# td-kwj-zp2023/webgpu-msm-twisted-edwards

Hardware: AMD Instinct MI355X
Metric: MSMs/sec at n=2^20 Twisted-Edwards BLS12 (pipelined throughput = 1000/ms_per_step; single-MSM latency in latency_ms) (higher is better)
Workload: dtype u32

## Files before the change

webgpu-msm-twisted-edwards_amd/csrc/curve.hpp:

```cpp
#pragma once
#include "field.hpp"

namespace te {

template <int N> struct ete_t { fel<N> x, y, z, t; };
using ete = ete_t<9>;

template <int N> struct pnt_t;
template <> struct pnt_t<9> { fel<9> hm, hp, dt; };
template <> struct pnt_t<14> { fel<14> hm, hp, dt, z; };
using pnt = pnt_t<9>;
struct pnt_aff377 { fel<14> hm, hp, dt; };

template <int N> TE_HD ete_t<N> ete_identity_t() { ete_t<N> r; r.x = fe_zero<N>(); r.y = fe_one<N>(); r.z = fe_one<N>(); r.t = fe_zero<N>(); return r; }
TE_HD ete ete_identity() { return ete_identity_t<9>(); }

TE_HD uint32_t mask_select(uint32_t m, uint32_t b, uint32_t a) {
#if defined(__HIP_DEVICE_COMPILE__)
  return __builtin_amdgcn_bitop3_b32(m, b, a, 0xCA);
#else
  return (b & m) | (a & ~m);
#endif
}
template <int N> TE_HD pnt_t<N> pnt_cneg(const pnt_t<N>& a, bool neg) {
  pnt_t<N> r = a; const fel<N> ndt = fe_neg<4>(a.dt);
  const uint32_t m = neg ? 0xffffffffu : 0u;
#pragma unroll
  for (int i = 0; i < N; i++) {
    r.hm.v[i] = mask_select(m, a.hp.v[i], a.hm.v[i]);
    r.hp.v[i] = mask_select(m, a.hm.v[i], a.hp.v[i]);
    r.dt.v[i] = mask_select(m, ndt.v[i], a.dt.v[i]);
  }
  return r;
}

TE_HD pnt_aff377 pnt_cneg(const pnt_aff377& a, bool neg) {
  pnt_aff377 r = a; const fel<14> ndt = fe_neg<4>(a.dt);
  const uint32_t m = neg ? 0xffffffffu : 0u;
#pragma unroll
  for (int i = 0; i < 14; i++) {
    r.hm.v[i] = mask_select(m, a.hp.v[i], a.hm.v[i]);
    r.hp.v[i] = mask_select(m, a.hm.v[i], a.hp.v[i]);
    r.dt.v[i] = mask_select(m, ndt.v[i], a.dt.v[i]);
  }
  return r;
}

template <bool MONT = false> TE_HD pnt pnt_from_affine_raw(const fp& x, const fp& y) {
  const fp k = MONT ? fp_R2_HALF_A() : fp_R2_HALF();
  const fp a[2] = {fp_sub<16>(y, x), fp_add(y, x)}, b[2] = {k, k};
  fp o[2];
  mont_mul_x<2>(a, b, o);
  pnt r;
  r.hm = o[0]; r.hp = o[1];
  r.dt = fp_mul_d(mont_mul(fp_add(o[1], o[0]), fp_sub<2>(o[0], o[1])));
  return r;
}

template <bool MONT = false> TE_HD pnt_t<14> pnt_from_sw377(const fel<14>& x, const fel<14>& y) {
  using namespace te377;
  const fq a1[3] = {x, y, x}, b1[3] = {MONT ? fq_S_R2_A() : fq_S_R2(), MONT ? fq_R2_A() : fq_R2(), MONT ? fq_F_R2_A() : fq_F_R2()};
  fq o1[3];
  fe_mul_x<3>(a1, b1, o1);
  const fq w = fe_norm(fe_add(o1[0], fq_SP1_MONT())), bb = fe_add(o1[0], fq_SM1_MONT()), aa = fe_norm(fe_add(o1[2], fq_F_MONT()));
  const fq a2[4] = {w, o1[1], o1[1], aa}, b2[4] = {aa, bb, w, bb};
  fq o2[4];
  fe_mul_x<4>(a2, b2, o2);
  pnt_t<14> r;
  r.hm = fe_norm(fe_sub<2>(o2[1], o2[0]));
  r.hp = fe_norm(fe_add(o2[1], o2[0]));
  r.z = fe_norm(fe_add(o2[2], o2[2]));
  r.dt = fe_mul(o2[3], fq_NEG_2D_MONT());
  return r;
}

template <int N> TE_HD ete_t<N> ete_close(const fel<N>& E, const fel<N>& H, const fel<N>& F, const fel<N>& G) {
  const fel<N> En = fe_norm_if_needed(E), Gn = fe_norm_if_needed(G);
  const fel<N> l[4] = {En, H, En, Gn}, rr[4] = {F, Gn, H, F};
  fel<N> o[4];
  fe_mul_x<4>(l, rr, o);
  ete_t<N> r;
  r.x = o[0]; r.y = o[1]; r.t = o[2]; r.z = o[3];
  return r;
}

TE_HD ete ete_madd(const ete& a, const pnt& b) {
  const fp in1[3] = {fp_sub<2>(a.y, a.x), fp_add(a.y, a.x), a.t}, in2[3] = {b.hm, b.hp, b.dt};
  fp abc[3];
  mont_mul_x<3>(in1, in2, abc);
  const fp &A = abc[0], &B = abc[1], &Cn = abc[2];
  return ete_close<9>(fp_sub<2>(B, A), fp_add(B, A), fp_add(a.z, Cn), fp_sub<2>(a.z, Cn));
}
TE_HD ete_t<14> ete_madd(const ete_t<14>& a, const pnt_t<14>& b) {
  const fel<14> in1[4] = {fe_sub<2>(a.y, a.x), fe_add(a.y, a.x), a.t, a.z}, in2[4] = {b.hm, b.hp, b.dt, b.z};
  fel<14> p[4];
  fe_mul_x<4>(in1, in2, p);
  const fel<14> &A = p[0], &B = p[1], &Cn = p[2], &D = p[3];
  return ete_close<14>(fe_sub<2>(B, A), fe_add(B, A), fe_add(D, Cn), fe_sub<2>(D, Cn));
}

TE_HD ete_t<14> ete_madd(const ete_t<14>& a, const pnt_aff377& b) {
  const fel<14> in1[3] = {fe_sub<2>(a.y, a.x), fe_add(a.y, a.x), a.t}, in2[3] = {b.hm, b.hp, b.dt};
  fel<14> p[3];
  fe_mul_x<3>(in1, in2, p);
  const fel<14> &A = p[0], &B = p[1], &Cn = p[2];
  return ete_close<14>(fe_sub<2>(B, A), fe_add(B, A), fe_add(a.z, Cn), fe_sub<2>(a.z, Cn));
}

TE_HD ete ete_from_pnt(const pnt& b) {
  const fp one = fp_R1();
  const fp E = fp_sub<2>(b.hp, b.hm), H = fp_add(b.hp, b.hm);
  const fp l[3] = {E, H, E}, rr[3] = {one, one, H};
  fp o[3];
  mont_mul_x<3>(l, rr, o);
  ete r;
  r.x = o[0]; r.y = o[1]; r.t = o[2]; r.z = one;
  return r;
}
TE_HD ete_t<14> ete_from_pnt(const pnt_t<14>& b) {
  const fel<14> En = fe_norm(fe_sub<2>(b.hp, b.hm)), H = fe_add(b.hp, b.hm);
  const fel<14> l[4] = {En, H, En, b.z}, rr[4] = {b.z, b.z, H, b.z};
  fel<14> o[4];
  fe_mul_x<4>(l, rr, o);
  ete_t<14> r;
  r.x = o[0]; r.y = o[1]; r.t = o[2]; r.z = o[3];
  return r;
}

TE_HD ete_t<14> ete_from_pnt(const pnt_aff377& b) {
  const fel<14> one = fe_one<14>();
  const fel<14> En = fe_norm(fe_sub<2>(b.hp, b.hm)), H = fe_add(b.hp, b.hm);
  const fel<14> l[3] = {En, H, En}, rr[3] = {one, one, H};
  fel<14> o[3];
  fe_mul_x<3>(l, rr, o);
  ete_t<14> r;
  r.x = o[0]; r.y = o[1]; r.t = o[2]; r.z = one;
  return r;
}

TE_HD ete ete_from_pair(const pnt& a, const pnt& b) {
  const fp one = fp_R1();
  const fp T1 = mont_mul(fp_add(a.hp, a.hm), fp_sub<2>(a.hp, a.hm));
  const fp in1[3] = {fp_add(a.hm, a.hm), fp_add(a.hp, a.hp), T1}, in2[3] = {b.hm, b.hp, b.dt};
  fp abc[3];
  mont_mul_x<3>(in1, in2, abc);
  const fp &A = abc[0], &B = abc[1], &Cn = abc[2];
  return ete_close<9>(fp_sub<2>(B, A), fp_add(B, A), fp_add(one, Cn), fp_sub<2>(one, Cn));
}
TE_HD ete_t<14> ete_from_pair(const pnt_aff377& a, const pnt_aff377& b) {
  const fel<14> one = fe_one<14>();
  const fel<14> T1 = fe_mul(fe_add(a.hp, a.hm), fe_norm(fe_sub<2>(a.hp, a.hm)));
  const fel<14> in1[3] = {fe_add(a.hm, a.hm), fe_add(a.hp, a.hp), T1}, in2[3] = {b.hm, b.hp, b.dt};
  fel<14> p[3];
  fe_mul_x<3>(in1, in2, p);
  const fel<14> &A = p[0], &B = p[1], &Cn = p[2];
  return ete_close<14>(fe_sub<2>(B, A), fe_add(B, A), fe_add(one, Cn), fe_sub<2>(one, Cn));
}
TE_HD ete_t<14> ete_from_pair(const pnt_t<14>& a, const pnt_t<14>& b) { return ete_madd(ete_from_pnt(a), b); }

template <int N> TE_HD ete_t<N> ete_add(const ete_t<N>& a, const ete_t<N>& b) {
  const fel<N> in1[4] = {fe_norm(fe_sub<2>(a.y, a.x)), fe_norm_if_needed(fe_add(a.y, a.x)), a.t, a.z};
  const fel<N> in2[4] = {fe_sub<2>(b.y, b.x), fe_add(b.y, b.x), b.t, b.z};
  fel<N> p1[4];
  fe_mul_x<4>(in1, in2, p1);
  const fel<N> &A = p1[0], &B = p1[1];
  const fel<N> C = fe_mul_k2d(p1[2]);
  const fel<N> D = fe_add(p1[3], p1[3]);
  const fel<N> E = fe_norm_if_needed(fe_sub<2>(B, A));
  const fel<N> H = fe_add(B, A);
  const fel<N> F = fe_norm(fe_sub<2>(D, C));
  const fel<N> G = fe_norm_if_needed(fe_add(D, C));
  const fel<N> l[4] = {E, H, E, F}, rr[4] = {F, G, H, G};
  fel<N> o[4];
  fe_mul_x<4>(l, rr, o);
  ete_t<N> r;
  r.x = o[0]; r.y = o[1]; r.t = o[2]; r.z = o[3];
  return r;
}

}
```

webgpu-msm-twisted-edwards_amd/csrc/kernels.hip.hpp:

```cpp
#pragma once
#include <hip/hip_runtime.h>
#include "curve.hpp"
#include "scalar_form.hpp"

namespace te {

#define TE_BATCH_MAX 8
struct batch_ptrs { const uint4* p[TE_BATCH_MAX]; };
struct batch_slabs { uint32_t s[TE_BATCH_MAX]; };

struct digits_params {
  uint32_t half[10];
  uint32_t zero_digit;
  uint32_t sc_stride;
  uint32_t n, nst;
  int num_windows;
  int w_first, w_step, nw_local;
  uint32_t half_code, logS, P, CH, chunk_len;
};

struct pnt_slot { uint4 q[8]; };
template <bool MONT = false>
__device__ __forceinline__ void prep_points_block(uint32_t blk, uint4* __restrict__ lds, const uint4* __restrict__ pts, pnt_slot* __restrict__ recs, uint32_t n) {
  const uint32_t t = threadIdx.x, base = blk * 256u;
// ... 363 lines not shown
      }
    }
    __syncthreads();
    for (uint32_t p = t; p < g.P; p += 512u) { run_base[p] += tile_cnt[p]; tile_cnt[p] = 0u; }
    __syncthreads();
  }
}

__global__ void __launch_bounds__(512) k_part_scatter(scatter_args a) {
  __shared__ uint32_t lds[TE_SCATTER_LDS_WORDS];
  part_scatter_block<false>(blockIdx.x, blockIdx.y, lds, a, index_args{});
}
__global__ void __launch_bounds__(512) k_part_scatter_indexed(scatter_args a, index_args x) {
  __shared__ uint32_t lds[TE_SCATTER_LDS_WORDS];
  part_scatter_block<true>(blockIdx.x, blockIdx.y, lds, a, x);
}

#ifndef TE_SCATTER_PREP_WAVES
#define TE_SCATTER_PREP_WAVES 8
#endif
__global__ void __launch_bounds__(512, TE_SCATTER_PREP_WAVES) k_part_scatter_prep(scatter_args a, uint32_t scatter_blocks, batch_ptrs in, batch_slabs row_slab,
                                                           pnt_slot* __restrict__ recs, uint32_t n, uint32_t prep_blocks_per_row, uint32_t prep_blocks) {
  __shared__ uint4 lds4[(TE_SCATTER_LDS_WORDS + 3u) / 4u > 256u * 8u ? (TE_SCATTER_LDS_WORDS + 3u) / 4u : 256u * 8u];
  const uint64_t tot = (uint64_t)scatter_blocks + prep_blocks, b = blockIdx.x;
  const uint32_t s_before = (uint32_t)(b * scatter_blocks / tot), s_after = (uint32_t)((b + 1u) * scatter_blocks / tot);
  if (s_after > s_before) {
    part_scatter_block<false>(s_before % a.g.CH, s_before / a.g.CH, reinterpret_cast<uint32_t*>(lds4), a, index_args{});
  } else {
    const uint32_t pb = (uint32_t)b - s_before, row = pb / prep_blocks_per_row, blk = pb - row * prep_blocks_per_row;
    prep_points_block(blk, lds4, in.p[row], recs + (size_t)row_slab.s[row] * n, n);
  }
}


struct piece_regs { uint4 k[5], ia[5], ib[5]; };
template <bool PK>
__device__ __forceinline__ void load_piece(const uint16_t* __restrict__ keys_row, const uint32_t* __restrict__ idx_row, uint32_t a, uint32_t b,
                                           uint32_t t, bool with_idx, piece_regs& r, uint32_t& head, uint32_t& total) {
  const uint32_t a_al = a & ~7u;
  head = a - a_al; total = head + (b - a);
  const uint32_t groups = (total + 7u) >> 3;
  const uint4* k4 = reinterpret_cast<const uint4*>(keys_row + a_al);
  const uint4* i4 = reinterpret_cast<const uint4*>(idx_row + a_al);
#pragma unroll
  for (int c = 0; c < 5; c++) {
    const uint32_t gi = min((uint32_t)c * 256u + t, groups - 1u);
    if (!PK) r.k[c] = k4[gi];
    if (PK || with_idx) { r.ia[c] = i4[2 * gi]; r.ib[c] = i4[2 * gi + 1]; }
  }
}
template <bool PK> __device__ __forceinline__ void piece_group(const piece_regs& r, int c, uint32_t (&kv)[8], uint32_t (&iv)[8]) {
  const uint32_t w[8] = {r.ia[c].x, r.ia[c].y, r.ia[c].z, r.ia[c].w, r.ib[c].x, r.ib[c].y, r.ib[c].z, r.ib[c].w};
  if (PK) {
#pragma unroll
    for (int e = 0; e < 8; e++) { kv[e] = ((w[e] >> 23) & 0xffu) | ((w[e] >> 31) << 15); iv[e] = w[e] & 0x7fffffu; }
  } else {
    unpack8(r.k[c], kv);
#pragma unroll
    for (int e = 0; e < 8; e++) iv[e] = w[e];
  }
}
static_assert(5u * 256u * 8u >= TE_L2_CAP + 8u, "five groups per thread hold a piece");

__device__ __forceinline__ bool l2_piece_of_block(uint32_t bx, const uint32_t* __restrict__ pc, uint32_t P, uint32_t overflow_pieces, uint32_t* sm, uint32_t* pj, uint32_t& p, uint32_t& j) {
  if (bx < P) { p = bx; j = 0u; return true; }
  const uint32_t t = threadIdx.x, x = bx - P;
  if (x >= overflow_pieces) return false;
  const uint32_t c = t < P ? pc[t] : 0u;
  const uint32_t ov = c ? (c + TE_L2_CAP - 1u) / TE_L2_CAP - 1u : 0u;
  uint32_t tot;
  const uint32_t ex = block_excl_scan(ov, sm, tot);
  if (x >= tot) return false;
  if (x >= ex && x < ex + ov) { pj[0] = t; pj[1] = x - ex + 1u; }
  __syncthreads();
  p = pj[0]; j = pj[1];
  __syncthreads();
  return true;
}

#define TE_COMBINE_SMALL 16u
#define TE_GIANT_RUN 256u
#define TE_SEG_INVALID 0xffffffffu
#define TE_HIST_COPIES 32u
struct plan_args {
  const uint32_t* part_start; const uint32_t* part_count; const uint32_t* seg_part_base;
  uint32_t *bucket_start, *bucket_cursor, *seg_base, *seg_bucket, *seg_lenv, *size_hist, *split_list;
  uint32_t* split_count;
  uint32_t* chunk_list;
  uint32_t seg_len, cap_w, chunk_cap;
};
struct plan_lds { uint32_t h[1024]; uint32_t sm[17]; uint32_t giant[256 * 3]; uint32_t n_giant; };
__device__ __forceinline__ uint32_t seg_plan_block(uint32_t p, uint32_t k, uint32_t cnt_in, const sort_geom& sg, const plan_args& a, plan_lds& L,
                                                   uint32_t pstart, uint32_t pcount, uint32_t sbase) {
  const uint32_t t = threadIdx.x, P = sg.P, S = sg.S, B = sg.B, seg_len = a.seg_len;
  uint32_t* const h = L.h; uint32_t* const sm = L.sm; uint32_t* const giant = L.giant;
  __syncthreads();
  for (uint32_t j = t; j < 1024u; j += 256u) h[j] = 0u;
  if (t == 0) L.n_giant = 0u;
  const bool mine = t < S;
  const uint32_t g = k * B + p * S + (mine ? t : 0u);
  const uint32_t cnt = mine ? cnt_in : 0u;
  const uint32_t nparts = mine ? max(1u, (cnt + seg_len - 1u) / seg_len) : 0u;
  uint32_t bt, bt2;
  const uint32_t ex = block_excl_scan(cnt, sm, bt);
  const uint32_t ex2 = block_excl_scan(nparts, sm, bt2);
  const uint32_t bs = pstart + ex, sb = sbase + ex2;
  if (mine) {
    a.bucket_start[g] = bs; a.bucket_cursor[g] = bs; a.seg_base[g] = sb;
    if (nparts <= TE_COMBINE_SMALL) {
      for (uint32_t part = 0; part < nparts; part++) {
        const uint32_t len = cnt > part * seg_len ? min(seg_len, cnt - part * seg_len) : 0u;
        a.seg_bucket[sb + part] = g; a.seg_lenv[sb + part] = len;
        atomicAdd(&h[min(len, 1023u)], 1u);
      }
      if (nparts > 1u) a.split_list[atomicAdd(&a.split_count[0], 1u)] = g;
    } else {
      const uint32_t j = atomicAdd(&L.n_giant, 1u);
      giant[3 * j] = g; giant[3 * j + 1] = sb; giant[3 * j + 2] = cnt;
      atomicAdd(&a.split_count[1], 1u);
    }
  }
  {
    const uint32_t first = sbase, used = bt2;
    const uint32_t cap = p + 1u == P ? (k + 1u) * a.cap_w - first : S + pcount / seg_len;
    for (uint32_t j = used + t; j < cap; j += 256u) { a.seg_bucket[first + j] = TE_SEG_INVALID; a.seg_lenv[first + j] = TE_SEG_INVALID; }
  }
  __syncthreads();
  const uint32_t ng = L.n_giant;
  for (uint32_t j = 0; j < ng; j++) {
    const uint32_t gg = giant[3 * j], sb0 = giant[3 * j + 1], c0 = giant[3 * j + 2];
    const uint32_t np = (c0 + seg_len - 1u) / seg_len;
    for (uint32_t part = t; part < np; part += 256u) {
      const uint32_t len = min(seg_len, c0 - part * seg_len);
      a.seg_bucket[sb0 + part] = gg; a.seg_lenv[sb0 + part] = len;
      atomicAdd(&h[min(len, 1023u)], 1u);
      if ((part & (TE_GIANT_RUN - 1u)) == 0) { const uint32_t ci = atomicAdd(&a.split_count[2], 1u); if (ci < a.chunk_cap) { a.chunk_list[2 * ci] = gg; a.chunk_list[2 * ci + 1] = part; } }
    }
  }
  __syncthreads();
  uint32_t* my_hist = a.size_hist + ((k * P + p) % TE_HIST_COPIES) * 1024u;
  for (uint32_t j = t; j < 1024u; j += 256u) if (h[j]) atomicAdd(&my_hist[j], h[j]);
  __syncthreads();
  return ex;
}

struct l2_args {
  const uint16_t* part_keys; const uint32_t* part_idx; const uint32_t* part_start; const uint32_t* part_count;
  uint32_t* bucket_count; uint32_t* sorted;
  uint32_t* part_ticket;
  sort_geom g; plan_args pa;
};
#define TE_L2A_LDS_WORDS (3u * 256u + 32u + TE_L2_LIST)
static_assert(sizeof(plan_lds) <= TE_L2_LIST * 4u, "the plan's LDS fits into the list area");
template <bool PK>
__global__ void __launch_bounds__(256, TE_L2_WAVES) k_l2_local(l2_args a) {
  __shared__ uint32_t lds[TE_L2A_LDS_WORDS];
  uint32_t* const cnt_s = lds; uint32_t* const off_s = lds + 256; uint32_t* const sm = lds + 768; uint32_t* const pj = lds + 768 + 17;
  uint32_t* const list = lds + 768 + 32;
  plan_lds& PL = *reinterpret_cast<plan_lds*>(list);
  const sort_geom& g = a.g;
  const uint32_t k = gridDim.y - 1u - blockIdx.y, t = threadIdx.x;
  const uint32_t extra = gridDim.x - g.P, bx = blockIdx.x < extra ? g.P + blockIdx.x : blockIdx.x - extra;
  const uint32_t* ps = a.part_start + k * g.P; const uint32_t* pc = a.part_count + k * g.P;
  uint32_t p, j;
  if (!l2_piece_of_block(bx, pc, g.P, bx < g.P ? 0u : a.part_count[gridDim.y * g.P + k], sm, pj, p, j)) return;
  const uint32_t cntp = pc[p], pb = ps[p], sbp = a.pa.seg_part_base[k * g.P + p];
  if (cntp == 0u) { (void)seg_plan_block(p, k, 0u, g, a.pa, PL, pb, cntp, sbp); return; }
  const bool single = cntp <= TE_L2_CAP;
  const uint32_t a0 = pb + j * TE_L2_CAP, b0 = min(pb + cntp, a0 + TE_L2_CAP);
  const uint16_t* keys_row = a.part_keys + (size_t)k * g.nst; const uint32_t* idx_row = a.part_idx + (size_t)k * g.nst;
  piece_regs r; uint32_t head, total;
  load_piece<PK>(keys_row, idx_row, a0, b0, t, single, r, head, total);
  cnt_s[t] = 0u;
  __syncthreads();
#pragma unroll
  for (int c = 0; c < 5; c++) {
    uint32_t kv[8], iv[8]; piece_group<PK>(r, c, kv, iv);
    const uint32_t e0 = ((uint32_t)c * 256u + t) * 8u;
#pragma unroll
    for (int e = 0; e < 8; e++) { const uint32_t pos = e0 + (uint32_t)e; if (pos >= head && pos < total) atomicAdd(&cnt_s[kv[e] & 0x7fffu], 1u); }
  }
  __syncthreads();
  const uint32_t c0 = cnt_s[t];
  const size_t gb = (size_t)k * g.B + (size_t)p * g.S + t;
  if (!single) {
    if (c0) atomicAdd(&a.bucket_count[gb], c0);
    wait_own_accesses();
    __syncthreads();
    if (t == 0) pj[2] = (handoff_arrive(&a.part_ticket[k * g.P + p]) + 1u == (cntp + TE_L2_CAP - 1u) / TE_L2_CAP) ? 1u : 0u;
    __syncthreads();
    if (pj[2]) (void)seg_plan_block(p, k, t < g.S ? ld_agent(a.bucket_count + gb) : 0u, g, a.pa, PL, pb, cntp, sbp);
    return;
  }
  if (t < g.S) a.bucket_count[gb] = c0;
  const uint32_t ex = seg_plan_block(p, k, c0, g, a.pa, PL, pb, cntp, sbp);
  if (t < g.S) a.pa.bucket_cursor[gb] = pb + ex + c0;
  off_s[t] = ex;
  __syncthreads();
#pragma unroll
  for (int c = 0; c < 5; c++) {
    uint32_t kv[8], iv[8]; piece_group<PK>(r, c, kv, iv);
    const uint32_t e0 = ((uint32_t)c * 256u + t) * 8u;
#pragma unroll
    for (int e = 0; e < 8; e++) {
      const uint32_t pos = e0 + (uint32_t)e;
      if (pos >= head && pos < total) list[atomicAdd(&off_s[kv[e] & 0x7fffu], 1u)] = iv[e] | ((kv[e] >> 15) << 31);
    }
  }
  __syncthreads();
  uint32_t* out = a.sorted + (size_t)k * g.n + pb;
  for (uint32_t s = t; s < cntp; s += 256u) out[s] = list[s];
}

#define TE_ORDER_REGS 32u
__device__ __forceinline__ void order_scatter_block(uint32_t ob, uint32_t nob, uint32_t* __restrict__ lds, const uint32_t* __restrict__ lenv, uint32_t ids,
                                                    const uint32_t* __restrict__ size_hist, uint32_t* __restrict__ rel_cursor,
                                                    uint32_t* __restrict__ order, uint32_t* __restrict__ num_segments, uint32_t max_len) {
  uint32_t* const h = lds; uint32_t* const base = lds + 1024; uint32_t* const sm = lds + 2048;
  const uint32_t per = (ids + nob - 1) / nob;
  const uint32_t lo = min(ids, ob * per), hi = min(ids, lo + per);
  const bool in_regs = per <= TE_ORDER_REGS * 256u;
  uint32_t lv[TE_ORDER_REGS];
  if (in_regs) {
#pragma unroll
    for (uint32_t j = 0; j < TE_ORDER_REGS; j++) { const uint32_t g = lo + j * 256u + threadIdx.x; lv[j] = g < hi ? lenv[g] : TE_SEG_INVALID; }
  }
  for (uint32_t j = threadIdx.x; j < 1024u; j += 256u) h[j] = 0;
  {
    uint32_t run = 0;
    for (uint32_t c = (1023u - min(max_len, 1023u)) >> 8; c < 4u; c++) {
      const uint32_t s = 1023u - (c * 256u + threadIdx.x);
      uint32_t part[TE_HIST_COPIES];
#pragma unroll
      for (uint32_t r = 0; r < TE_HIST_COPIES; r++) part[r] = size_hist[r * 1024u + s];
      uint32_t cnt_s = 0;
#pragma unroll
      for (uint32_t r = 0; r < TE_HIST_COPIES; r++) cnt_s += part[r];
      uint32_t bt;
      const uint32_t ex = block_excl_scan(cnt_s, sm, bt);
      base[s] = run + ex;
      run += bt;
    }
    if (ob == 0 && threadIdx.x == 0) *num_segments = run;
  }
  __syncthreads();
  if (in_regs) {
#pragma unroll
    for (uint32_t j = 0; j < TE_ORDER_REGS; j++) if (lv[j] != TE_SEG_INVALID) atomicAdd(&h[min(lv[j], 1023u)], 1u);
  } else {
    for (uint32_t g = lo + threadIdx.x; g < hi; g += 256u) { const uint32_t l = lenv[g]; if (l != TE_SEG_INVALID) atomicAdd(&h[min(l, 1023u)], 1u); }
  }
  __syncthreads();
  for (uint32_t j = threadIdx.x; j < 1024u; j += 256u) { base[j] += h[j] ? atomicAdd(&rel_cursor[j], h[j]) : 0u; h[j] = 0; }
  __syncthreads();
  if (in_regs) {
#pragma unroll
    for (uint32_t j = 0; j < TE_ORDER_REGS; j++) {
      if (lv[j] == TE_SEG_INVALID) continue;
      const uint32_t sz = min(lv[j], 1023u);
      order[base[sz] + atomicAdd(&h[sz], 1u)] = lo + j * 256u + threadIdx.x;
    }
  } else {
    for (uint32_t g = lo + threadIdx.x; g < hi; g += 256u) {
      const uint32_t l = lenv[g];
      if (l == TE_SEG_INVALID) continue;
      const uint32_t sz = min(l, 1023u);
      order[base[sz] + atomicAdd(&h[sz], 1u)] = g;
    }
  }
}

#define TE_PLACE_LDS_WORDS (4u * 256u + TE_L2_LIST + TE_L2_LIST / 4u + 2u + 17u)
template <bool PK>
__device__ __forceinline__ void l2_place_piece(uint32_t p, uint32_t k, uint32_t a0, uint32_t b0, uint32_t* __restrict__ lds,
                                               const uint16_t* __restrict__ part_keys, const uint32_t* __restrict__ part_idx,
                                               uint32_t* __restrict__ bucket_cursor, uint32_t* __restrict__ sorted, const sort_geom& g) {
  uint32_t* const cnt_s = lds; uint32_t* const lex_s = lds + 256; uint32_t* const off_s = lds + 512; uint32_t* const gbase_s = lds + 768;
  uint32_t* const list = lds + 1024;
  uint8_t* const list_b = reinterpret_cast<uint8_t*>(list + TE_L2_LIST);
  uint32_t* const sm = list + TE_L2_LIST + TE_L2_LIST / 4u + 2u;
  const uint32_t t = threadIdx.x, len = b0 - a0;
  const uint16_t* keys_row = part_keys + (size_t)k * g.nst; const uint32_t* idx_row = part_idx + (size_t)k * g.nst;
  uint32_t* out = sorted + (size_t)k * g.n;
  cnt_s[t] = 0u;
  __syncthreads();
  piece_regs r; uint32_t head, total;
  load_piece<PK>(keys_row, idx_row, a0, b0, t, true, r, head, total);
#pragma unroll
  for (int c = 0; c < 5; c++) {
    uint32_t kv[8], iv[8]; piece_group<PK>(r, c, kv, iv);
    const uint32_t e0 = ((uint32_t)c * 256u + t) * 8u;
#pragma unroll
    for (int e = 0; e < 8; e++) { const uint32_t pos = e0 + (uint32_t)e; if (pos >= head && pos < total) atomicAdd(&cnt_s[kv[e] & 0x7fffu], 1u); }
  }
  __syncthreads();
  wave0_excl_scan(cnt_s, lex_s, 256u, &sm[16]);
  {
    const uint32_t c0 = cnt_s[t];
    gbase_s[t] = c0 ? atomicAdd(&bucket_cursor[(size_t)k * g.B + (size_t)p * g.S + t], c0) : 0u;
  }
  __syncthreads();
  off_s[t] = lex_s[t];
  gbase_s[t] -= lex_s[t];
  __syncthreads();
#pragma unroll
  for (int c = 0; c < 5; c++) {
    uint32_t kv[8], iv[8]; piece_group<PK>(r, c, kv, iv);
    const uint32_t e0 = ((uint32_t)c * 256u + t) * 8u;
#pragma unroll
    for (int e = 0; e < 8; e++) {
      const uint32_t pos = e0 + (uint32_t)e;
      if (pos >= head && pos < total) {
        const uint32_t b = kv[e] & 0x7fffu;
        const uint32_t slot = atomicAdd(&off_s[b], 1u);
        list[slot] = iv[e] | ((kv[e] >> 15) << 31); list_b[slot] = (uint8_t)b;
      }
    }
  }
  __syncthreads();
  for (uint32_t s = t; s < len; s += 256u) out[gbase_s[list_b[s]] + s] = list[s];
}

struct order_args { const uint32_t* lenv; uint32_t ids; const uint32_t* size_hist; uint32_t* rel_cursor; uint32_t* order; uint32_t* num_segments; uint32_t order_cols, max_len; };
template <bool PK>
__global__ void __launch_bounds__(256, TE_L2_WAVES) k_l2_place_order(const uint16_t* __restrict__ part_keys, const uint32_t* __restrict__ part_idx,
                                                           const uint32_t* __restrict__ part_start, const uint32_t* __restrict__ part_count,
                                                           uint32_t* __restrict__ bucket_cursor, uint32_t* __restrict__ sorted, sort_geom g, order_args oa) {
  __shared__ uint32_t lds[TE_PLACE_LDS_WORDS];
  if (blockIdx.x < oa.order_cols) {
    order_scatter_block(blockIdx.y * oa.order_cols + blockIdx.x, gridDim.y * oa.order_cols, lds, oa.lenv, oa.ids, oa.size_hist, oa.rel_cursor, oa.order, oa.num_segments, oa.max_len);
    return;
  }
  const uint32_t k = gridDim.y - 1u - blockIdx.y;
  const uint32_t px = blockIdx.x - oa.order_cols, extra = gridDim.x - oa.order_cols - g.P, bx = px < extra ? g.P + px : px - extra;
  const uint32_t* pc = part_count + k * g.P;
  uint32_t p, j;
  if (!l2_piece_of_block(bx, pc, g.P, bx < g.P ? 0u : part_count[gridDim.y * g.P + k], lds, lds + 32, p, j)) return;
  const uint32_t cntp = pc[p], pb = part_start[k * g.P + p];
  if (cntp <= TE_L2_CAP) return;
  const uint32_t a0 = pb + j * TE_L2_CAP;
  l2_place_piece<PK>(p, k, a0, min(pb + cntp, a0 + TE_L2_CAP), lds, part_keys, part_idx, bucket_cursor, sorted, g);
}

template <int N> struct geo {
  static constexpr uint32_t PW = 4u * N;
  static constexpr uint32_t PQ = PW / 4u;
  static constexpr uint32_t RW = N == 9 ? 27u : 4u * N;
  static constexpr uint32_t SQ = N == 9 ? 8u : N;
  static constexpr uint32_t LQ = (RW + 3u) / 4u;
};
template <int N> struct rec_slot { uint4 q[geo<N>::SQ]; };
static_assert(sizeof(rec_slot<9>) == sizeof(pnt_slot) && sizeof(rec_slot<14>) == 224, "record slots");

template <int N> __device__ __forceinline__ pnt_t<N> load_pnt(const rec_slot<N>* __restrict__ recs, uint32_t entry) {
  const uint4* q = recs[entry & 0x7fffffffu].q;
  constexpr uint32_t LQ = geo<N>::LQ;
  uint4 u[LQ];
#pragma unroll
  for (uint32_t j = 0; j < LQ; j++) u[j] = q[j];
  uint32_t w[4 * LQ];
#pragma unroll
  for (uint32_t j = 0; j < LQ; j++) { w[4 * j] = u[j].x; w[4 * j + 1] = u[j].y; w[4 * j + 2] = u[j].z; w[4 * j + 3] = u[j].w; }
  pnt_t<N> r;
#pragma unroll
  for (int j = 0; j < N; j++) { r.hm.v[j] = w[j]; r.hp.v[j] = w[N + j]; r.dt.v[j] = w[2 * N + j]; }
  if constexpr (N == 14) {
#pragma unroll
    for (int j = 0; j < N; j++) r.z.v[j] = w[3 * N + j];
  }
  return r;
}
template <int N> __device__ __forceinline__ void store_pnt(rec_slot<N>* dst, const pnt_t<N>& r) {
  uint32_t w[4 * geo<N>::SQ];
#pragma unroll
  for (uint32_t j = 0; j < 4 * geo<N>::SQ; j++) w[j] = 0u;
#pragma unroll
  for (int j = 0; j < N; j++) { w[j] = r.hm.v[j]; w[N + j] = r.hp.v[j]; w[2 * N + j] = r.dt.v[j]; }
  if constexpr (N == 14) {
#pragma unroll
    for (int j = 0; j < N; j++) w[3 * N + j] = r.z.v[j];
  }
#pragma unroll
  for (uint32_t j = 0; j < geo<N>::SQ; j++) dst->q[j] = make_uint4(w[4 * j], w[4 * j + 1], w[4 * j + 2], w[4 * j + 3]);
}
template <int N> __device__ __forceinline__ void store_ete(ete_t<N>* dst, const ete_t<N>& a) {
  uint32_t w[4 * N];
#pragma unroll
  for (int j = 0; j < N; j++) { w[j] = a.x.v[j]; w[N + j] = a.y.v[j]; w[2 * N + j] = a.z.v[j]; w[3 * N + j] = a.t.v[j]; }
  uint4* o = reinterpret_cast<uint4*>(dst);
#pragma unroll
  for (int j = 0; j < N; j++) o[j] = make_uint4(w[4 * j], w[4 * j + 1], w[4 * j + 2], w[4 * j + 3]);
}
template <int N> __device__ __forceinline__ ete_t<N> load_ete(const ete_t<N>* src) {
  const uint4* q = reinterpret_cast<const uint4*>(src);
  uint32_t w[4 * N];
#pragma unroll
  for (int j = 0; j < N; j++) { const uint4 u = q[j]; w[4 * j] = u.x; w[4 * j + 1] = u.y; w[4 * j + 2] = u.z; w[4 * j + 3] = u.w; }
  ete_t<N> a;
#pragma unroll
  for (int j = 0; j < N; j++) { a.x.v[j] = w[j]; a.y.v[j] = w[N + j]; a.z.v[j] = w[2 * N + j]; a.t.v[j] = w[3 * N + j]; }
  return a;
}

struct __attribute__((aligned(8))) rec_aff377 { uint32_t w[42]; };
struct __attribute__((aligned(8))) u4a8 { uint32_t v[4]; };
struct __attribute__((aligned(8))) u2a8 { uint32_t v[2]; };
static_assert(sizeof(rec_aff377) == 168, "affine record slot");
__device__ __forceinline__ pnt_aff377 load_pnt_aff377(const rec_aff377* __restrict__ recs, uint32_t entry) {
  const uint32_t* base = recs[entry & 0x7fffffffu].w;
  u4a8 u[10];
#pragma unroll
  for (int j = 0; j < 10; j++) u[j] = reinterpret_cast<const u4a8*>(base)[j];
  const u2a8 t = *reinterpret_cast<const u2a8*>(base + 40);
  uint32_t w[42];
#pragma unroll
  for (int j = 0; j < 10; j++) { w[4 * j] = u[j].v[0]; w[4 * j + 1] = u[j].v[1]; w[4 * j + 2] = u[j].v[2]; w[4 * j + 3] = u[j].v[3]; }
  w[40] = t.v[0]; w[41] = t.v[1];
  pnt_aff377 r;
#pragma unroll
  for (int j = 0; j < 14; j++) { r.hm.v[j] = w[j]; r.hp.v[j] = w[14 + j]; r.dt.v[j] = w[28 + j]; }
  return r;
}
__device__ __forceinline__ void store_pnt_aff377(rec_aff377* dst, const pnt_aff377& r) {
#pragma unroll
  for (int j = 0; j < 14; j++) { dst->w[j] = r.hm.v[j]; dst->w[14 + j] = r.hp.v[j]; dst->w[28 + j] = r.dt.v[j]; }
}
template <int N, int RK> struct rec_kind;
template <int N> struct rec_kind<N, 0> {
  using slot = rec_slot<N>; using pnt = pnt_t<N>;
  static __device__ __forceinline__ pnt load(const slot* __restrict__ recs, uint32_t e) { return load_pnt<N>(recs, e); }
};
template <> struct rec_kind<14, 1> {
  using slot = rec_aff377; using pnt = pnt_aff377;
  static __device__ __forceinline__ pnt load(const slot* __restrict__ recs, uint32_t e) { return load_pnt_aff377(recs, e); }
};

struct __attribute__((aligned(4))) idx4 { uint32_t v[4]; };
#define TE_CLK_SLOTS 64u
#define TE_IDX_STRIP 16u
template <int N, int RK = 0>
__global__ void __attribute__((amdgpu_flat_work_group_size(1, 256), amdgpu_waves_per_eu(N == 9 ? 3 : 2, N == 9 ? 3 : 2))) k_accumulate(const typename rec_kind<N, RK>::slot* __restrict__ recs, const uint32_t* __restrict__ sorted,
                                                    const uint32_t* __restrict__ bucket_start, const uint32_t* __restrict__ bucket_count,
                                                    const uint32_t* __restrict__ seg_base, const uint32_t* __restrict__ seg_bucket,
                                                    const uint32_t* __restrict__ seg_lenv, const uint32_t* __restrict__ order,
                                                    const uint32_t* __restrict__ num_segments, ete_t<N>* __restrict__ buckets,
                                                    ete_t<N>* __restrict__ seg_out, uint32_t n, uint32_t logB, uint32_t seg_len, uint32_t ids, uint32_t onto,
                                                    uint32_t win_per_msm, batch_slabs slabs, unsigned long long* __restrict__ clk) {
  __shared__ __attribute__((aligned(16))) uint32_t idx_strip[256 * TE_IDX_STRIP];
  using RT = rec_kind<N, RK>; using P = typename RT::pnt;
  unsigned long long* const slot = clk ? clk + (blockIdx.x & (TE_CLK_SLOTS - 1u)) : nullptr;
  const unsigned long long t0_wall = clk ? (unsigned long long)wall_clock64() : 0ull, t0_core = clk ? (unsigned long long)clock64() : 0ull;
  if (clk && threadIdx.x == 0) atomicMax(slot, ~t0_wall);
  const uint32_t gid = blockIdx.x * 256u + threadIdx.x;
  if (gid >= (order ? *num_segments : ids)) return;
  const uint32_t sgm = order ? order[gid] : gid;
  const uint32_t g = seg_bucket[sgm];
  if (g == TE_SEG_INVALID) return;
  const uint32_t k = g >> logB;
  recs += (size_t)slabs.s[k / win_per_msm] * n;
  const uint32_t part = sgm - seg_base[g];
  const uint32_t cnt = seg_lenv[sgm];
  const uint32_t* lst = sorted + (size_t)k * n + bucket_start[g] + part * seg_len;
  ete_t<N> acc = (onto && part == 0u) ? load_ete<N>(buckets + g) : ete_identity_t<N>();
  if (cnt) {
    const uint32_t last = cnt - 1u;
    uint32_t j0 = 0;
    uint32_t e = lst[0], e_n = lst[min(1u, last)];
    const uint32_t e_2 = lst[min(2u, last)], e_3 = lst[min(3u, last)];
    P cur = RT::load(recs, e);
    if (!(onto && part == 0u)) {
      const P first = pnt_cneg(cur, (e >> 31) != 0u);
      if (cnt >= 2u) {
        const P second = pnt_cneg(RT::load(recs, e_n), (e_n >> 31) != 0u);
        e = e_2; e_n = e_3;
        cur = RT::load(recs, e);
        acc = ete_from_pair(first, second);
        j0 = 2;
      } else {
        acc = ete_from_pnt(first);
        j0 = 1;
      }
    }
    uint32_t* const strip = idx_strip + threadIdx.x * TE_IDX_STRIP;
    auto refill = [&](uint32_t pos) {
      const idx4* src = reinterpret_cast<const idx4*>(lst + pos);
      idx4* dst = reinterpret_cast<idx4*>(strip);
#pragma unroll
      for (uint32_t h = 0; h < TE_IDX_STRIP / 4u; h += 2u) {
        const idx4 v0 = src[h], v1 = src[h + 1u];
        dst[h] = v0; dst[h + 1u] = v1;
      }
    };
    if (((j0 + 2u) & (TE_IDX_STRIP - 1u)) != 0u) refill((j0 + 2u) & ~(TE_IDX_STRIP - 1u));
    P rec_b;
    uint32_t j = j0;
    for (; j + 2u < cnt; j += 2u) {
      const uint32_t pn = j + 2u;
      if ((pn & (TE_IDX_STRIP - 1u)) == 0u) refill(pn);
      const uint2 e_nn = *reinterpret_cast<const uint2*>(strip + (pn & (TE_IDX_STRIP - 1u)));
      rec_b = RT::load(recs, e_n);
      acc = ete_madd(acc, pnt_cneg(cur, (e >> 31) != 0u));
      __builtin_amdgcn_sched_barrier(0);
      cur = RT::load(recs, e_nn.x);
      acc = ete_madd(acc, pnt_cneg(rec_b, (e_n >> 31) != 0u));
      e = e_nn.x; e_n = e_nn.y;
    }
    if (j < cnt) {
      const bool two = j + 1u < cnt;
      rec_b = RT::load(recs, two ? e_n : e);
      acc = ete_madd(acc, pnt_cneg(cur, (e >> 31) != 0u));
      if (two) acc = ete_madd(acc, pnt_cneg(rec_b, (e_n >> 31) != 0u));
    }
  }
  const bool whole = bucket_count[g] <= seg_len;
  store_ete<N>(whole ? buckets + g : seg_out + sgm, acc);
  if (clk && (uint32_t)__lane_id() == (uint32_t)__ffsll((long long)__ballot(1)) - 1u) {
    const unsigned long long t1_wall = (unsigned long long)wall_clock64(), t1_core = (unsigned long long)clock64();
    atomicMax(slot + TE_CLK_SLOTS, t1_wall);
    atomicAdd(slot + 2u * TE_CLK_SLOTS, t1_core - t0_core); atomicAdd(slot + 3u * TE_CLK_SLOTS, t1_wall - t0_wall);
  }
}

template <int N> struct sum_job_t {
  const ete_t<N>* in; ete_t<N>* out;
  uint32_t n_out;
  uint32_t K, inner;
  uint32_t in_per_window, out_per_window;
};
template <int N> struct sum_jobs_t { sum_job_t<N> j[4]; };
template <int N> __device__ __forceinline__ ete_t<N> pair_swap(const ete_t<N>& a) {
  ete_t<N> r;
#pragma unroll
  for (int i = 0; i < N; i++) {
    r.x.v[i] = (uint32_t)__builtin_amdgcn_mov_dpp((int)a.x.v[i], 0xb1, 0xf, 0xf, true);
    r.y.v[i] = (uint32_t)__builtin_amdgcn_mov_dpp((int)a.y.v[i], 0xb1, 0xf, 0xf, true);
    r.z.v[i] = (uint32_t)__builtin_amdgcn_mov_dpp((int)a.z.v[i], 0xb1, 0xf, 0xf, true);
    r.t.v[i] = (uint32_t)__builtin_amdgcn_mov_dpp((int)a.t.v[i], 0xb1, 0xf, 0xf, true);
  }
  return r;
}
template <int N, bool PAIR>
__global__ void __launch_bounds__(256, N == 9 ? 2 : 1) k_sum_groups(sum_jobs_t<N> js, uint32_t nw) {
  const sum_job_t<N>& j = js.j[blockIdx.y];
  constexpr uint32_t TPO = PAIR ? 2u : 1u;
  const uint32_t total = j.n_out * nw * TPO, Kt = j.K / TPO;
  for (uint32_t gt = blockIdx.x * 256u + threadIdx.x; gt < total; gt += gridDim.x * 256u) {
    const uint32_t g = gt / TPO, half = gt % TPO;
    const uint32_t k = g / j.n_out, o = g - k * j.n_out;
    const uint32_t outer = o / j.inner, q = o - outer * j.inner;
    const ete_t<N>* src = j.in + (size_t)k * j.in_per_window + ((size_t)outer * j.K + (size_t)half * Kt) * j.inner + q;
    ete_t<N> acc = load_ete<N>(src);
    if (Kt > 1u) {
      ete_t<N> nxt = load_ete<N>(src + (size_t)j.inner);
      for (uint32_t t = 1; t < Kt; t++) {
        const ete_t<N> cur = nxt;
        if (t + 1 < Kt) nxt = load_ete<N>(src + (size_t)(t + 1) * j.inner);
        acc = ete_add<N>(acc, cur);
      }
    }
    if (PAIR) {
      const ete_t<N> other = pair_swap<N>(acc);
      acc = ete_add<N>(acc, other);
      if (half != 0u) continue;
    }
    store_ete<N>(j.out + (size_t)k * j.out_per_window + o, acc);
  }
}

template <int N> __device__ __forceinline__ fel<N> quad_bcast(const fel<N>& v, const int k) {
  fel<N> r;
#pragma unroll
  for (int i = 0; i < N; i++) {
    const int x = (int)v.v[i];
    int y;
    switch (k) {
      case 0: y = __builtin_amdgcn_mov_dpp(x, 0x00, 0xf, 0xf, true); break;
      case 1: y = __builtin_amdgcn_mov_dpp(x, 0x55, 0xf, 0xf, true); break;
      case 2: y = __builtin_amdgcn_mov_dpp(x, 0xaa, 0xf, 0xf, true); break;
      default: y = __builtin_amdgcn_mov_dpp(x, 0xff, 0xf, 0xf, true); break;
    }
    r.v[i] = (uint32_t)y;
  }
  return r;
}
template <int N> __device__ __forceinline__ fel<N> quad_swap1(const fel<N>& v) {
  fel<N> r;
#pragma unroll
  for (int i = 0; i < N; i++) r.v[i] = (uint32_t)__builtin_amdgcn_mov_dpp((int)v.v[i], 0xb1, 0xf, 0xf, true);
  return r;
}
template <int N> __device__ __forceinline__ fel<N> fp_select(bool c, const fel<N>& a, const fel<N>& b) {
  fel<N> r;
#pragma unroll
  for (int i = 0; i < N; i++) r.v[i] = c ? a.v[i] : b.v[i];
  return r;
}
template <int N> __device__ __forceinline__ fel<N> fe_pick(uint32_t m, const fel<N>& b, const fel<N>& a) {
  fel<N> r;
#pragma unroll
  for (int i = 0; i < N; i++) r.v[i] = mask_select(m, b.v[i], a.v[i]);
  return r;
}
template <int N> __device__ __forceinline__ fel<N> ete_add_team(const fel<N>& m1, const fel<N>& m2, const uint32_t q) {
  const fel<N> o1 = quad_swap1<N>(m1), o2 = quad_swap1<N>(m2);
  const fel<N> u0 = fe_norm(fe_sub<2>(o1, m1)), v0 = fe_sub<2>(o2, m2);
  const fel<N> u1 = fe_norm_if_needed(fe_add(m1, o1)), v1 = fe_add(m2, o2);
  const uint32_t q0 = q == 0u ? ~0u : 0u, q1 = q == 1u ? ~0u : 0u, q2 = q == 2u ? ~0u : 0u, q3 = q == 3u ? ~0u : 0u;
  const fel<N> u = fe_pick<N>(q0, u0, fe_pick<N>(q1, u1, m1));
  const fel<N> v = fe_pick<N>(q0, v0, fe_pick<N>(q1, v1, m2));
  const fel<N> s1 = fe_mul(u, v);
  const fel<N> s2 = fe_mul_k2d(s1);
  const fel<N> val = fe_pick<N>(q2, s2, fe_pick<N>(q3, fe_add(s1, s1), s1));
  const fel<N> A = quad_bcast<N>(val, 0), B = quad_bcast<N>(val, 1), C = quad_bcast<N>(val, 2), D = quad_bcast<N>(val, 3);
  const fel<N> E = fe_norm_if_needed(fe_sub<2>(B, A)), H = fe_add(B, A), F = fe_norm(fe_sub<2>(D, C)), G = fe_norm_if_needed(fe_add(D, C));
  const fel<N> uu = fe_pick<N>(q0 | q2, E, fe_pick<N>(q1, H, F));
  const fel<N> vv = fe_pick<N>(q0, F, fe_pick<N>(q2, H, G));
  return fe_mul(uu, vv);
}
template <int N> __device__ __forceinline__ uint32_t team_word(uint32_t q) { return (q == 0 ? 0u : q == 1 ? 1u : q == 2 ? 3u : 2u) * N; }
template <int N> __device__ __forceinline__ fel<N> load_coord(const uint32_t* p) { fel<N> r;
#pragma unroll
  for (int i = 0; i < N; i++) r.v[i] = p[i];
  return r; }
template <int N> __device__ __forceinline__ void store_coord(uint32_t* p, const fel<N>& a) {
#pragma unroll
  for (int i = 0; i < N; i++) p[i] = a.v[i];
}
template <int N> __device__ __forceinline__ fel<N> identity_coord(uint32_t q) { return (q == 1 || q == 3) ? fe_one<N>() : fe_zero<N>(); }
template <int N> __device__ __forceinline__ const uint32_t* words(const ete_t<N>* p) { return reinterpret_cast<const uint32_t*>(p); }
template <int N> __device__ __forceinline__ uint32_t* words(ete_t<N>* p) { return reinterpret_cast<uint32_t*>(p); }

template <int N> __device__ __forceinline__ fel<N> load_coord_agent(const uint32_t* p) { fel<N> r;
#pragma unroll
  for (int i = 0; i < N; i++) r.v[i] = ld_agent(p + i);
  return r; }
template <int N> __device__ __forceinline__ void store_coord_agent(uint32_t* p, const fel<N>& a) {
#pragma unroll
  for (int i = 0; i < N; i++) st_agent(p + i, a.v[i]);
}
template <int N, bool COHERENT = false> __device__ __forceinline__ fel<N> block_sum_points(const ete_t<N>* __restrict__ src, uint32_t stride, uint32_t cnt, uint32_t* lds) {
  constexpr uint32_t PW = geo<N>::PW;
  const uint32_t i = threadIdx.x >> 2, q = threadIdx.x & 3u, w = team_word<N>(q);
  fel<N> acc = identity_coord<N>(q);
  auto fetch = [&](uint32_t j) { return COHERENT ? load_coord_agent<N>(words<N>(src + (size_t)j * stride) + w) : load_coord<N>(words<N>(src + (size_t)j * stride) + w); };
  if (i < cnt) {
    acc = fetch(i);
    fel<N> nxt = fetch(min(i + 64u, cnt - 1u));
    for (uint32_t j = i + 64u; j < cnt; j += 64u) {
      const fel<N> cur = nxt;
      if (j + 64u < cnt) nxt = fetch(j + 64u);
      acc = ete_add_team<N>(acc, cur, q);
    }
  }
  for (uint32_t s = 32; s > 0; s >>= 1) {
    if (s >= cnt) continue;
    if (i >= s && i < 2 * s) store_coord<N>(lds + (size_t)i * PW + w, acc);
    __syncthreads();
    if (((threadIdx.x & ~63u) >> 2) < s) {
      const bool act = i < s && i + s < cnt;
      const fel<N> other = act ? load_coord<N>(lds + (size_t)(i + s) * PW + w) : identity_coord<N>(q);
      const fel<N> sum = ete_add_team<N>(acc, other, q);
      acc = fp_select<N>(act, sum, acc);
    }
    __syncthreads();
// ... 405 lines not shown
```

Measured before the change: 1142.

## Track accumulator sign to replace per-point conditional negation with lazy flips

The bucket accumulation loop now keeps the accumulator in (y-x, y+x, z, t) form and tracks a sign flag. Instead of conditionally negating each loaded point, it negates the accumulator only when the sign changes, using register swaps and a negated t. The final sign is folded into the last subtraction via fe_diff. The local L2 sort also counts positive and negative entries separately and places them in contiguous runs, so sign flips become rare. The cost is extra sort bookkeeping and more complex correctness reasoning.

```diff
diff --git a/webgpu-msm-twisted-edwards_amd/csrc/curve.hpp b/webgpu-msm-twisted-edwards_amd/csrc/curve.hpp
--- a/webgpu-msm-twisted-edwards_amd/csrc/curve.hpp
+++ b/webgpu-msm-twisted-edwards_amd/csrc/curve.hpp
@@ -84,32 +84,61 @@
   return r;
 }
 
-TE_HD ete ete_madd(const ete& a, const pnt& b) {
-  const fp in1[3] = {fp_sub<2>(a.y, a.x), fp_add(a.y, a.x), a.t}, in2[3] = {b.hm, b.hp, b.dt};
+template <int N> struct ete_uv_t { fel<N> u, v, z, t; };
+template <int N> TE_HD ete_uv_t<N> ete_open(const ete_t<N>& a) {
+  ete_uv_t<N> r;
+  r.u = fe_sub<2>(a.y, a.x); r.v = fe_add(a.y, a.x); r.z = a.z; r.t = a.t;
+  return r;
+}
+template <int N> TE_HD void ete_uv_neg(ete_uv_t<N>& a) {
+#pragma unroll
+  for (int i = 0; i < N; i++) {
+#if defined(__HIP_DEVICE_COMPILE__)
+    asm("v_swap_b32 %0, %1" : "+v"(a.u.v[i]), "+v"(a.v.v[i]));
+#else
+    const uint32_t w = a.u.v[i]; a.u.v[i] = a.v.v[i]; a.v.v[i] = w;
+#endif
+  }
+  a.t = fe_neg<2>(a.t);
+}
+template <bool SGN, int N> TE_HD fel<N> fe_diff(const fel<N>& b, const fel<N>& a, bool neg) {
+  if constexpr (!SGN) return fe_sub<2>(b, a);
+  else {
+    const uint32_t m = neg ? 0xffffffffu : 0u;
+    fel<N> hi, lo;
+#pragma unroll
+    for (int i = 0; i < N; i++) { hi.v[i] = mask_select(m, a.v[i], b.v[i]); lo.v[i] = mask_select(m, b.v[i], a.v[i]); }
+    return fe_sub<2>(hi, lo);
+  }
+}
+template <bool SGN = false> TE_HD ete ete_madd_raw(const ete_uv_t<9>& a, const pnt& b, bool neg = false) {
+  const fp in1[3] = {a.u, a.v, a.t}, in2[3] = {b.hm, b.hp, b.dt};
   fp abc[3];
   mont_mul_x<3>(in1, in2, abc);
   const fp &A = abc[0], &B = abc[1], &Cn = abc[2];
-  return ete_close<9>(fp_sub<2>(B, A), fp_add(B, A), fp_add(a.z, Cn), fp_sub<2>(a.z, Cn));
-}
-TE_HD ete_t<14> ete_madd(const ete_t<14>& a, const pnt_t<14>& b) {
-  const fel<14> in1[4] = {fe_sub<2>(a.y, a.x), fe_add(a.y, a.x), a.t, a.z}, in2[4] = {b.hm, b.hp, b.dt, b.z};
+  return ete_close<9>(fe_diff<SGN, 9>(B, A, neg), fp_add(B, A), fp_add(a.z, Cn), fp_sub<2>(a.z, Cn));
+}
+template <bool SGN = false> TE_HD ete_t<14> ete_madd_raw(const ete_uv_t<14>& a, const pnt_t<14>& b, bool neg = false) {
+  const fel<14> in1[4] = {a.u, a.v, a.t, a.z}, in2[4] = {b.hm, b.hp, b.dt, b.z};
   fel<14> p[4];
   fe_mul_x<4>(in1, in2, p);
   const fel<14> &A = p[0], &B = p[1], &Cn = p[2], &D = p[3];
-  return ete_close<14>(fe_sub<2>(B, A), fe_add(B, A), fe_add(D, Cn), fe_sub<2>(D, Cn));
-}
-
-TE_HD ete_t<14> ete_madd(const ete_t<14>& a, const pnt_aff377& b) {
-  const fel<14> in1[3] = {fe_sub<2>(a.y, a.x), fe_add(a.y, a.x), a.t}, in2[3] = {b.hm, b.hp, b.dt};
+  return ete_close<14>(fe_diff<SGN, 14>(B, A, neg), fe_add(B, A), fe_add(D, Cn), fe_sub<2>(D, Cn));
+}
+template <bool SGN = false> TE_HD ete_t<14> ete_madd_raw(const ete_uv_t<14>& a, const pnt_aff377& b, bool neg = false) {
+  const fel<14> in1[3] = {a.u, a.v, a.t}, in2[3] = {b.hm, b.hp, b.dt};
   fel<14> p[3];
   fe_mul_x<3>(in1, in2, p);
   const fel<14> &A = p[0], &B = p[1], &Cn = p[2];
-  return ete_close<14>(fe_sub<2>(B, A), fe_add(B, A), fe_add(a.z, Cn), fe_sub<2>(a.z, Cn));
-}
-
-TE_HD ete ete_from_pnt(const pnt& b) {
+  return ete_close<14>(fe_diff<SGN, 14>(B, A, neg), fe_add(B, A), fe_add(a.z, Cn), fe_sub<2>(a.z, Cn));
+}
+TE_HD ete ete_madd(const ete& a, const pnt& b) { return ete_madd_raw(ete_open<9>(a), b); }
+TE_HD ete_t<14> ete_madd(const ete_t<14>& a, const pnt_t<14>& b) { return ete_madd_raw(ete_open<14>(a), b); }
+TE_HD ete_t<14> ete_madd(const ete_t<14>& a, const pnt_aff377& b) { return ete_madd_raw(ete_open<14>(a), b); }
+
+template <bool SGN = false> TE_HD ete ete_from_pnt(const pnt& b, bool neg = false) {
   const fp one = fp_R1();
-  const fp E = fp_sub<2>(b.hp, b.hm), H = fp_add(b.hp, b.hm);
+  const fp E = fe_diff<SGN, 9>(b.hp, b.hm, neg), H = fp_add(b.hp, b.hm);
   const fp l[3] = {E, H, E}, rr[3] = {one, one, H};
   fp o[3];
   mont_mul_x<3>(l, rr, o);
@@ -117,8 +146,8 @@
   r.x = o[0]; r.y = o[1]; r.t = o[2]; r.z = one;
   return r;
 }
-TE_HD ete_t<14> ete_from_pnt(const pnt_t<14>& b) {
-  const fel<14> En = fe_norm(fe_sub<2>(b.hp, b.hm)), H = fe_add(b.hp, b.hm);
+template <bool SGN = false> TE_HD ete_t<14> ete_from_pnt(const pnt_t<14>& b, bool neg = false) {
+  const fel<14> En = fe_norm(fe_diff<SGN, 14>(b.hp, b.hm, neg)), H = fe_add(b.hp, b.hm);
   const fel<14> l[4] = {En, H, En, b.z}, rr[4] = {b.z, b.z, H, b.z};
   fel<14> o[4];
   fe_mul_x<4>(l, rr, o);
@@ -127,9 +156,9 @@
   return r;
 }
 
-TE_HD ete_t<14> ete_from_pnt(const pnt_aff377& b) {
+template <bool SGN = false> TE_HD ete_t<14> ete_from_pnt(const pnt_aff377& b, bool neg = false) {
   const fel<14> one = fe_one<14>();
-  const fel<14> En = fe_norm(fe_sub<2>(b.hp, b.hm)), H = fe_add(b.hp, b.hm);
+  const fel<14> En = fe_norm(fe_diff<SGN, 14>(b.hp, b.hm, neg)), H = fe_add(b.hp, b.hm);
   const fel<14> l[3] = {En, H, En}, rr[3] = {one, one, H};
   fel<14> o[3];
   fe_mul_x<3>(l, rr, o);
@@ -138,25 +167,27 @@
   return r;
 }
 
-TE_HD ete ete_from_pair(const pnt& a, const pnt& b) {
+template <bool SGN = false> TE_HD ete ete_from_pair(const pnt& a, const pnt& b, bool neg = false) {
   const fp one = fp_R1();
   const fp T1 = mont_mul(fp_add(a.hp, a.hm), fp_sub<2>(a.hp, a.hm));
   const fp in1[3] = {fp_add(a.hm, a.hm), fp_add(a.hp, a.hp), T1}, in2[3] = {b.hm, b.hp, b.dt};
   fp abc[3];
   mont_mul_x<3>(in1, in2, abc);
   const fp &A = abc[0], &B = abc[1], &Cn = abc[2];
-  return ete_close<9>(fp_sub<2>(B, A), fp_add(B, A), fp_add(one, Cn), fp_sub<2>(one, Cn));
-}
-TE_HD ete_t<14> ete_from_pair(const pnt_aff377& a, const pnt_aff377& b) {
+  return ete_close<9>(fe_diff<SGN, 9>(B, A, neg), fp_add(B, A), fp_add(one, Cn), fp_sub<2>(one, Cn));
+}
+template <bool SGN = false> TE_HD ete_t<14> ete_from_pair(const pnt_aff377& a, const pnt_aff377& b, bool neg = false) {
   const fel<14> one = fe_one<14>();
   const fel<14> T1 = fe_mul(fe_add(a.hp, a.hm), fe_norm(fe_sub<2>(a.hp, a.hm)));
   const fel<14> in1[3] = {fe_add(a.hm, a.hm), fe_add(a.hp, a.hp), T1}, in2[3] = {b.hm, b.hp, b.dt};
   fel<14> p[3];
   fe_mul_x<3>(in1, in2, p);
   const fel<14> &A = p[0], &B = p[1], &Cn = p[2];
-  return ete_close<14>(fe_sub<2>(B, A), fe_add(B, A), fe_add(one, Cn), fe_sub<2>(one, Cn));
-}
-TE_HD ete_t<14> ete_from_pair(const pnt_t<14>& a, const pnt_t<14>& b) { return ete_madd(ete_from_pnt(a), b); }
+  return ete_close<14>(fe_diff<SGN, 14>(B, A, neg), fe_add(B, A), fe_add(one, Cn), fe_sub<2>(one, Cn));
+}
+template <bool SGN = false> TE_HD ete_t<14> ete_from_pair(const pnt_t<14>& a, const pnt_t<14>& b, bool neg = false) {
+  return ete_madd_raw<SGN>(ete_open<14>(ete_from_pnt(a)), b, neg);
+}
 
 template <int N> TE_HD ete_t<N> ete_add(const ete_t<N>& a, const ete_t<N>& b) {
   const fel<N> in1[4] = {fe_norm(fe_sub<2>(a.y, a.x)), fe_norm_if_needed(fe_add(a.y, a.x)), a.t, a.z};
diff --git a/webgpu-msm-twisted-edwards_amd/csrc/kernels.hip.hpp b/webgpu-msm-twisted-edwards_amd/csrc/kernels.hip.hpp
--- a/webgpu-msm-twisted-edwards_amd/csrc/kernels.hip.hpp
+++ b/webgpu-msm-twisted-edwards_amd/csrc/kernels.hip.hpp
@@ -539,6 +539,7 @@
 };
 #define TE_L2A_LDS_WORDS (3u * 256u + 32u + TE_L2_LIST)
 static_assert(sizeof(plan_lds) <= TE_L2_LIST * 4u, "the plan's LDS fits into the list area");
+static_assert(TE_L2_CAP < 65536u, "k_l2_local counts a bucket's positive and negative entries in the halves of one word");
 template <bool PK>
 __global__ void __launch_bounds__(256, TE_L2_WAVES) k_l2_local(l2_args a) {
   __shared__ uint32_t lds[TE_L2A_LDS_WORDS];
@@ -565,10 +566,10 @@
     uint32_t kv[8], iv[8]; piece_group<PK>(r, c, kv, iv);
     const uint32_t e0 = ((uint32_t)c * 256u + t) * 8u;
 #pragma unroll
-    for (int e = 0; e < 8; e++) { const uint32_t pos = e0 + (uint32_t)e; if (pos >= head && pos < total) atomicAdd(&cnt_s[kv[e] & 0x7fffu], 1u); }
-  }
-  __syncthreads();
-  const uint32_t c0 = cnt_s[t];
+    for (int e = 0; e < 8; e++) { const uint32_t pos = e0 + (uint32_t)e; if (pos >= head && pos < total) atomicAdd(&cnt_s[kv[e] & 0x7fffu], 1u << ((kv[e] >> 15) << 4)); }
+  }
+  __syncthreads();
+  const uint32_t c_pos = cnt_s[t] & 0xffffu, c0 = c_pos + (cnt_s[t] >> 16);
   const size_t gb = (size_t)k * g.B + (size_t)p * g.S + t;
   if (!single) {
     if (c0) atomicAdd(&a.bucket_count[gb], c0);
@@ -582,7 +583,7 @@
   if (t < g.S) a.bucket_count[gb] = c0;
   const uint32_t ex = seg_plan_block(p, k, c0, g, a.pa, PL, pb, cntp, sbp);
   if (t < g.S) a.pa.bucket_cursor[gb] = pb + ex + c0;
-  off_s[t] = ex;
+  off_s[t] = ex; off_s[256u + t] = ex + c_pos;
   __syncthreads();
 #pragma unroll
   for (int c = 0; c < 5; c++) {
@@ -591,7 +592,7 @@
 #pragma unroll
     for (int e = 0; e < 8; e++) {
       const uint32_t pos = e0 + (uint32_t)e;
-      if (pos >= head && pos < total) list[atomicAdd(&off_s[kv[e] & 0x7fffu], 1u)] = iv[e] | ((kv[e] >> 15) << 31);
+      if (pos >= head && pos < total) list[atomicAdd(&off_s[(kv[e] & 0x7fffu) + ((kv[e] >> 15) << 8)], 1u)] = iv[e] | ((kv[e] >> 15) << 31);
     }
   }
   __syncthreads();
@@ -849,6 +850,7 @@
   const uint32_t cnt = seg_lenv[sgm];
   const uint32_t* lst = sorted + (size_t)k * n + bucket_start[g] + part * seg_len;
   ete_t<N> acc = (onto && part == 0u) ? load_ete<N>(buckets + g) : ete_identity_t<N>();
+  bool flipped = false;
   if (cnt) {
     const uint32_t last = cnt - 1u;
     uint32_t j0 = 0;
@@ -856,15 +858,17 @@
     const uint32_t e_2 = lst[min(2u, last)], e_3 = lst[min(3u, last)];
     P cur = RT::load(recs, e);
     if (!(onto && part == 0u)) {
-      const P first = pnt_cneg(cur, (e >> 31) != 0u);
+      flipped = (e >> 31) != 0u;
+      const bool ends = cnt <= 2u;
       if (cnt >= 2u) {
-        const P second = pnt_cneg(RT::load(recs, e_n), (e_n >> 31) != 0u);
+        const P second = pnt_cneg(RT::load(recs, e_n), ((e_n ^ e) >> 31) != 0u);
         e = e_2; e_n = e_3;
+        const P first = cur;
         cur = RT::load(recs, e);
-        acc = ete_from_pair(first, second);
+        acc = ete_from_pair<true>(first, second, ends && flipped);
         j0 = 2;
       } else {
-        acc = ete_from_pnt(first);
+        acc = ete_from_pnt<true>(cur, flipped);
         j0 = 1;
       }
     }
@@ -879,24 +883,38 @@
       }
     };
     if (((j0 + 2u) & (TE_IDX_STRIP - 1u)) != 0u) refill((j0 + 2u) & ~(TE_IDX_STRIP - 1u));
-    P rec_b;
-    uint32_t j = j0;
-    for (; j + 2u < cnt; j += 2u) {
-      const uint32_t pn = j + 2u;
-      if ((pn & (TE_IDX_STRIP - 1u)) == 0u) refill(pn);
-      const uint2 e_nn = *reinterpret_cast<const uint2*>(strip + (pn & (TE_IDX_STRIP - 1u)));
-      rec_b = RT::load(recs, e_n);
-      acc = ete_madd(acc, pnt_cneg(cur, (e >> 31) != 0u));
-      __builtin_amdgcn_sched_barrier(0);
-      cur = RT::load(recs, e_nn.x);
-      acc = ete_madd(acc, pnt_cneg(rec_b, (e_n >> 31) != 0u));
-      e = e_nn.x; e_n = e_nn.y;
-    }
-    if (j < cnt) {
-      const bool two = j + 1u < cnt;
-      rec_b = RT::load(recs, two ? e_n : e);
-      acc = ete_madd(acc, pnt_cneg(cur, (e >> 31) != 0u));
-      if (two) acc = ete_madd(acc, pnt_cneg(rec_b, (e_n >> 31) != 0u));
+    ete_uv_t<N> uv = ete_open<N>(acc);
+    auto sign_to = [&](uint32_t entry) {
+      const bool s = (entry >> 31) != 0u;
+      if (s != flipped) { ete_uv_neg<N>(uv); flipped = s; }
+    };
+    if (j0 < cnt) {
+      P rec_b;
+      uint32_t j = j0;
+      for (; j + 2u < cnt; j += 2u) {
+        const uint32_t pn = j + 2u;
+        if ((pn & (TE_IDX_STRIP - 1u)) == 0u) refill(pn);
+        const uint2 e_nn = *reinterpret_cast<const uint2*>(strip + (pn & (TE_IDX_STRIP - 1u)));
+        rec_b = RT::load(recs, e_n);
+        sign_to(e);
+        uv = ete_open<N>(ete_madd_raw(uv, cur));
+        __builtin_amdgcn_sched_barrier(0);
+        cur = RT::load(recs, e_nn.x);
+        sign_to(e_n);
+        uv = ete_open<N>(ete_madd_raw(uv, rec_b));
+        e = e_nn.x; e_n = e_nn.y;
+      }
+      {
+        const bool two = j + 1u < cnt;
+        rec_b = RT::load(recs, two ? e_n : e);
+        sign_to(e);
+        acc = ete_madd_raw<true>(uv, cur, !two && flipped);
+        if (two) {
+          uv = ete_open<N>(acc);
+          sign_to(e_n);
+          acc = ete_madd_raw<true>(uv, rec_b, flipped);
+        }
+      }
     }
   }
   const bool whole = bucket_count[g] <= seg_len;
```

Result: faster. 1154 (median of 6 runs) (+1.1%).
